# jhqxxx/aha

Hardware: AMD Instinct MI355X
Metric: decode tokens/s (greedy, batch 1) -- Qwen3-VL-8B, 1x1024^2 image + 512-token prompt; prefill tok/s alongside (higher is better)
Workload: dtype bf16; 1 GPU; qwen3vl8b; image=1024, kv_len_mid=2024, replicas=1, loop=device-resident greedy loop

## Files before the change

### aha_amd/_lib.py

```python
from __future__ import annotations

import ctypes as C
import os

_HERE = os.path.dirname(os.path.abspath(__file__))
LIB_PATH = os.path.join(_HERE, "csrc", "libaha_hip.so")

AHA_BF16, AHA_F16, AHA_F32, AHA_U32, AHA_U8 = 0, 1, 2, 3, 4
AHA_ARCH_QWEN3, AHA_ARCH_QWEN3VL, AHA_ARCH_QWEN3ASR = 0, 1, 2
ACT_NONE, ACT_GELU_TANH, ACT_GELU_ERF, ACT_SILU, ACT_SILU_MUL_PAIRS = 0, 1, 2, 3, 4


AHA_SAMPLE_HAS_TOP_P, AHA_SAMPLE_HAS_TOP_K = 1, 2
AHA_SAMPLE_NEED_LOGITS = 1


class SamplingParams(C.Structure):
    _fields_ = [
        ("temperature", C.c_float), ("top_p", C.c_float), ("top_k", C.c_int32), ("repeat_penalty", C.c_float),
        ("repeat_last_n", C.c_int32), ("flags", C.c_uint32), ("seed", C.c_uint64),
    ]


AHA_ENGINE_EV_FIRST, AHA_ENGINE_EV_STOP, AHA_ENGINE_EV_LENGTH, AHA_ENGINE_EV_CANCELLED = 1, 2, 4, 8
# ... 117 lines not shown
                                            C.c_int64]),
    "aha_hip_debug_resample_taps": (C.c_int64, [C.c_int32, C.c_int32, C.POINTER(C.c_float), C.c_int64, C.POINTER(C.c_int32),
                                                C.POINTER(C.c_int32)]),
    "aha_hip_audio_resample": (C.c_int64, [_P, C.POINTER(C.c_float), C.c_int64, C.c_int32, C.c_int32, C.c_int32,
                                           C.POINTER(C.c_float), C.c_int64]),
    "aha_hip_cache_len": (C.c_size_t, [_P]),
    "aha_hip_debug_steps_executed": (C.c_int64, [_P]),
    "aha_hip_debug_graph_step": (C.c_int, [_P, C.c_int32, C.POINTER(C.c_double), C.POINTER(C.c_double)]),
    "aha_hip_kv_export": (C.c_int, [_P, _P, C.c_size_t, C.POINTER(C.c_size_t), C.POINTER(C.c_size_t), C.POINTER(C.c_int64)]),
    "aha_hip_kv_import": (C.c_int, [_P, _P, C.c_size_t, C.c_int32, C.c_int32, C.c_int32, C.c_int32, C.c_size_t, C.c_int64]),
    "aha_hip_set_profiling": (C.c_int, [_P, C.c_int]),
    "aha_hip_get_profile": (C.c_int, [_P, C.c_char_p, C.POINTER(C.c_double), C.POINTER(C.c_int64),
                                      C.POINTER(C.c_double), C.POINTER(C.c_double)]),
    "aha_hip_debug_scramble_pages": (C.c_int, [_P, C.c_int]),
    "aha_hip_debug_attn_decode_form": (C.c_int, [_P]),
    "aha_hip_debug_last_hidden": (C.c_int, [_P, C.POINTER(C.c_float), C.c_size_t]),
    "aha_hip_debug_image_embeds": (C.c_int, [_P, C.c_int, C.POINTER(C.c_float), C.c_size_t]),
    "aha_hip_rmsnorm": (C.c_int, [_P, _P, _P, C.c_int64, C.c_int32, C.c_float, _P]),
    "aha_hip_gemv": (C.c_int, [_P, _P, _P, C.c_int32, C.c_int32, _P, C.c_float, _P, _P]),
    "aha_hip_gemv_gate_up": (C.c_int, [_P, _P, _P, _P, C.c_int32, C.c_int32, _P, C.c_float, _P]),
    "aha_hip_gemm": (C.c_int, [_P, _P, _P, C.c_int32, C.c_int32, C.c_int32, C.c_int32, C.c_int32, C.c_int32, _P, _P,
                               C.c_int32, _P]),
    "aha_hip_qknorm_rope": (C.c_int, [_P, _P, _P, _P, _P, _P, _P, _P, C.c_int32, C.c_int32, C.c_int32, C.c_int32,
                                      C.c_float, C.c_float, _P]),
    "aha_hip_attn_decode": (C.c_int, [_P, _P, _P, _P, C.c_int32, C.c_int32, C.c_int32, C.c_int32, C.c_float, _P]),
    "aha_hip_attn_prefill": (C.c_int, [_P, _P, _P, _P, C.c_int32, C.c_int32, C.c_int32, C.c_int32, C.c_int32,
                                       C.c_int32, C.c_int32, C.c_float, _P]),
    "aha_hip_debug_attn_prefill_segs": (C.c_int, [_P, _P, _P, _P, C.c_int32, C.c_int32, _P, C.c_int32, C.c_int32, C.c_float, _P]),
    "aha_hip_debug_prefill_rope": (C.c_int, [_P, _P, _P, _P, _P, _P, _P, C.c_int32, C.c_int32, C.c_int32, C.c_int32, C.c_int32, C.c_float,
                                             C.c_int32, C.c_int32, C.c_int32, _P, _P, C.c_int32, _P, _P, _P]),
# ... 121 lines not shown
```

### aha_amd/csrc/attn_decode_body.h

```cpp
#pragma once
#include <type_traits>
#include "attn_common.h"

namespace aha {

constexpr int ATTN_DECODE_NW = 4;
constexpr int ATTN_DECODE_MO_ROW = 132;
constexpr int ATTN_DECODE_FUSED_LDS = 16 * 128 * 2 + 128 * 2 + 128 * 2 + ATTN_DECODE_NW * 16 * ATTN_DECODE_MO_ROW * 4 + 2 * ATTN_DECODE_NW * 16 * 4;

__device__ __forceinline__ float split_sum16(const float (&v)[16]) {
#pragma clang fp contract(off)
  float t[8];
#pragma unroll
  for (int j = 0; j < 8; ++j) t[j] = v[j] + v[j + 8];
#pragma unroll
  for (int j = 0; j < 4; ++j) t[j] = t[j] + t[j + 4];
  const float c0 = t[0] + t[2], c1 = t[1] + t[3];
  return c0 + c1;
}

template <bool APPEND = true, bool LINEAR = false>
__device__ __forceinline__ bool attn_decode_fused_body(const AttnDecodeFusedArgs& a, char* smem, const int kvhd, const int split,
                                                       const int nsplit) {
  constexpr int NW = ATTN_DECODE_NW, NT = NW * 64;
  bf16_t* qs = reinterpret_cast<bf16_t*>(smem);
  bf16_t* ksn = qs + 16 * 128;
  bf16_t* vsn = ksn + 128;
  constexpr int MO_ROW = ATTN_DECODE_MO_ROW, MO_WAVE = 16 * MO_ROW;
  float* mo = reinterpret_cast<float*>(vsn + 128);
  float* mm = mo + NW * MO_WAVE;
  float* mlz = mm + NW * 16;
  const int tid = (int)threadIdx.x;
  const int wave = __builtin_amdgcn_readfirstlane(tid >> 6);
  const int lane = tid & 63, G = lane >> 4, c = lane & 15;
  const int g = a.nh / a.kvh;
  const int nunits = nsplit * NW, unit = split * NW + wave;
  const int L = a.kv_len_v, slot_new = a.kv_start_v;
  const int L_old = L - 1;
  const int npages = (L_old + KV_PAGE_TOKENS - 1) / KV_PAGE_TOKENS;

  const int tslot = (kvhd == 0 && split == 0) ? 0 : (kvhd == 0 && split == nsplit - 1 ? 1 : -1);
  auto stamp = [&](int k) {
    if (a.trace != nullptr && tslot >= 0 && tid == 0) a.trace[tslot * 6 + k] = wall_clock64();
  };
  stamp(0);

  const bf16_t* qkv = (const bf16_t*)a.qkv;
  const bool p_is_k = wave == g;
  const bool p_have = wave <= g;
  const bf16_t* p_src = p_is_k ? qkv + (int64_t)(a.nh + kvhd) * 128 : qkv + (int64_t)(kvhd * g + min(wave, g - 1)) * 128;
  const bf16_t* p_nw = (const bf16_t*)(p_is_k ? a.k_norm_w : a.q_norm_w);
  const bf16_t px0 = p_src[lane], px1 = p_src[lane + 64];
  const bf16_t pw0 = p_nw[lane], pw1 = p_nw[lane + 64];
  const float cs = a.rope[lane], sn = a.rope[64 + lane];
  bf16_t vnew = 0;
  if (tid < 128) vnew = qkv[(int64_t)(a.nh + a.kvh + kvhd) * 128 + tid];

  u32x4_t kf[4][4], vf[8][2];
  typedef const __attribute__((address_space(1))) char* gchar_t;
  const uint32_t l_off = (uint32_t)lane * 16;
  auto load_k = [&](uint64_t base) {
    gchar_t kb = reinterpret_cast<gchar_t>(base + (uint64_t)kvhd * KV_PAGE_TOKENS * 256);
#pragma unroll
    for (int sub = 0; sub < 4; ++sub)
#pragma unroll
      for (int k4 = 0; k4 < 4; ++k4)
        kf[sub][k4] = __builtin_nontemporal_load(reinterpret_cast<gptr16_t>(kb + (sub * 4 + k4) * 1024 + l_off));
  };
  auto load_v = [&](uint64_t base) {
    gchar_t vb = reinterpret_cast<gchar_t>(base + (uint64_t)a.kvh * KV_PAGE_TOKENS * 256 + (uint64_t)kvhd * 128 * (KV_PAGE_TOKENS * 2));
#pragma unroll
    for (int ds = 0; ds < 8; ++ds)
#pragma unroll
      for (int kk = 0; kk < 2; ++kk)
        vf[ds][kk] = __builtin_nontemporal_load(reinterpret_cast<gptr16_t>(vb + (ds * 2 + kk) * 1024 + l_off));
  };
  uint64_t my_pages = 0;
  auto fetch_page_ptrs = [&](int first_it) {
    if (LINEAR) return;
    const int pg = unit + (first_it + lane) * nunits;
    my_pages = pg < npages ? (uint64_t)(a.kv.page_ptrs[pg] + a.kv.layer_off) : 0;
  };
  auto page_base = [&](int i) {
    if (LINEAR) return a.lin_page0 + (uint64_t)((int64_t)(unit + i * nunits) * a.lin_step);
    const uint32_t lo = __builtin_amdgcn_readlane((uint32_t)my_pages, i & 63), hi = __builtin_amdgcn_readlane((uint32_t)(my_pages >> 32), i & 63);
    return ((uint64_t)hi << 32) | lo;
  };
  fetch_page_ptrs(0);
  int page = unit, it = 0;
  if (page < npages) {
    const uint64_t b0 = page_base(0);
    __builtin_amdgcn_sched_barrier(0);
    load_k(b0);
    __builtin_amdgcn_sched_barrier(0);
    load_v(b0);
    __builtin_amdgcn_sched_barrier(0);
  }

  {
    auto norm_rope = [&](bf16_t bx0, bf16_t bx1, bf16_t bw0, bf16_t bw1, bf16_t* dst) {
      float x0 = bf2f(bx0), x1 = bf2f(bx1);
      const float ss = wave_sum(fmaf(x0, x0, x1 * x1));
      const float rinv = 1.0f / sqrtf(ss / 128.0f + a.eps);
      x0 = rbf(x0 * rinv * bf2f(bw0));
      x1 = rbf(x1 * rinv * bf2f(bw1));
      const bf16_t y0 = f2bf(rbf(x0 * cs) + rbf(-x1 * sn));
      const bf16_t y1 = f2bf(rbf(x1 * cs) + rbf(x0 * sn));
      dst[lane] = y0;
      dst[lane + 64] = y1;
    };
    if (p_have) norm_rope(px0, px1, pw0, pw1, p_is_k ? ksn : qs + wave * 128);
    for (int hs = wave + NW; hs <= g; hs += NW) {
      const bool is_k = hs == g;
      const bf16_t* src = is_k ? qkv + (int64_t)(a.nh + kvhd) * 128 : qkv + (int64_t)(kvhd * g + hs) * 128;
      const bf16_t* nw = (const bf16_t*)(is_k ? a.k_norm_w : a.q_norm_w);
      norm_rope(src[lane], src[lane + 64], nw[lane], nw[lane + 64], is_k ? ksn : qs + hs * 128);
    }
    if (tid < 128) vsn[tid] = vnew;
  }
  __syncthreads();
  stamp(1);
  if (APPEND && split == 0) {
    typedef __attribute__((address_space(1))) bf16_t* gbf_t;
    const int pg = slot_new / KV_PAGE_TOKENS, t = slot_new % KV_PAGE_TOKENS;
    const uint64_t base = LINEAR ? a.lin_page0 + (uint64_t)((int64_t)pg * a.lin_step) : (uint64_t)(a.kv.page_ptrs[pg] + a.kv.layer_off);
    gbf_t kd = reinterpret_cast<gbf_t>(base) + (int64_t)kvhd * KV_PAGE_TOKENS * 128;
    gbf_t vd = reinterpret_cast<gbf_t>(base) + (int64_t)a.kvh * KV_PAGE_TOKENS * 128 + (int64_t)kvhd * 128 * KV_PAGE_TOKENS;
    for (int i = tid; i < 128; i += NT) {
      kd[kpage_elem(t, i, 4)] = ksn[i];
      vd[vpage_elem(t, i)] = vsn[i];
    }
  }

  bf16x8_t qf[4];
#pragma unroll
  for (int k4 = 0; k4 < 4; ++k4) {
    u32x4_t v = *reinterpret_cast<const u32x4_t*>(qs + min(c, g - 1) * 128 + k4 * 32 + G * 8);
    if (c >= g) v = u32x4_t{0u, 0u, 0u, 0u};
    qf[k4] = as_frag(v);
  }
  float m = -INFINITY, l = 0.f;
  f32x4_t o[8];
#pragma unroll
// ... 20 lines not shown
    float alpha;
    bf16x8_t pf[2];
    const int t0 = page * KV_PAGE_TOKENS;
    softmax_tile(st, a.scale, [&](int t) { return t0 + t < L_old; }, G, m, l, alpha, pf);
#pragma unroll
    for (int ds = 0; ds < 8; ++ds) {
      o[ds] *= alpha;
#pragma unroll
      for (int kk = 0; kk < 2; ++kk) o[ds] = mfma16(as_frag(vf[ds][kk]), pf[kk], o[ds]);
    }
    __builtin_amdgcn_sched_barrier(0);
    if (MORE) load_v(nb);
    __builtin_amdgcn_sched_barrier(0);
    page += nunits;
  };
  if (page < npages) {
    while (page + nunits < npages) do_page(std::true_type{});
    do_page(std::false_type{});
  }
  stamp(2);
  if (unit == 0) {
    float dot = 0.f;
    const u32x4_t* qr = reinterpret_cast<const u32x4_t*>(qs + min(c, g - 1) * 128 + G * 32);
    const u32x4_t* kr = reinterpret_cast<const u32x4_t*>(ksn + G * 32);
    u32x4_t qv[4], kv4[4];
#pragma unroll
    for (int j = 0; j < 4; ++j) {
      qv[j] = qr[j];
      kv4[j] = kr[j];
    }
#pragma unroll
    for (int j = 0; j < 16; ++j) {
      const uint32_t qw = qv[j >> 2][j & 3], kw = kv4[j >> 2][j & 3];
      dot = fmaf(__uint_as_float(qw << 16), __uint_as_float(kw << 16), dot);
      dot = fmaf(__uint_as_float(qw & 0xffff0000u), __uint_as_float(kw & 0xffff0000u), dot);
    }
// ... 2 lines not shown
    const float m_new = fmaxf(m, s);
    const float alpha = __expf(m - m_new);
    const float p = rbf(__expf(s - m_new));
    l = l * alpha + (G == 0 ? __expf(s - m_new) : 0.f);
    m = m_new;
#pragma unroll
    for (int ds = 0; ds < 8; ++ds) {
      const uint2 vv = *reinterpret_cast<const uint2*>(vsn + ds * 16 + G * 4);
      o[ds][0] = fmaf(p, __uint_as_float(vv.x << 16), o[ds][0] * alpha);
      o[ds][1] = fmaf(p, __uint_as_float(vv.x & 0xffff0000u), o[ds][1] * alpha);
      o[ds][2] = fmaf(p, __uint_as_float(vv.y << 16), o[ds][2] * alpha);
      o[ds][3] = fmaf(p, __uint_as_float(vv.y & 0xffff0000u), o[ds][3] * alpha);
    }
  }
  l = group_sum(l);

  {
    float* wo = mo + wave * MO_WAVE + c * MO_ROW + G * 4;
#pragma unroll
    for (int ds = 0; ds < 8; ++ds) *reinterpret_cast<f32x4_t*>(wo + ds * 16) = o[ds];
    if (G == 0) {
      mm[wave * 16 + c] = m;
      mlz[wave * 16 + c] = l;
    }
  }
  __syncthreads();
  const bool single = nsplit == 1;
  const auto rsrc_w = __builtin_amdgcn_make_buffer_rsrc(a.part_o, 0, (int)((size_t)nsplit * a.nh * 128 * 4), 0x00020000);
  for (int item = tid; item < g * 32; item += NT) {
    const int q = item >> 5, d0 = (item & 31) * 4;
// ... 155 lines not shown
```

### aha_amd/csrc/capi.hip

```cpp
#include <math.h>
#include <string.h>

#include <algorithm>
#include <map>
#include <memory>
#include <mutex>
#include <numeric>
#include <vector>

#include "common.h"
#include "model.h"
#include "sampler.h"
#include "audio.h"
#include "vision.h"

namespace aha {
const char* last_error_cstr();
}
using namespace aha;

#define API_GUARD_BEGIN try {
#define API_GUARD_END                                   \
  }                                                     \
  catch (const std::exception& e) {                     \
// ... 147 lines not shown
}

int aha_hip_last_logits(aha_model* m, float* logits_out) {
  API_GUARD_BEGIN
  if (!m || !logits_out) {
    set_error("null argument");
    return AHA_ERR_INVALID;
  }
  return model_last_logits(m, logits_out);
  API_GUARD_END
}

size_t aha_hip_cache_len(const aha_model* m) { return m ? m->cache_len : 0; }
int64_t aha_hip_debug_steps_executed(const aha_model* m) { return m ? m->steps_executed : 0; }
int aha_hip_debug_attn_decode_form(const aha_model* m) { return m ? m->last_attn_form : -1; }
int aha_hip_debug_graph_step(aha_model* m, int32_t replays, double* us_launches, double* us_graph) {
  if (!m) return AHA_ERR_INVALID;
  API_GUARD_BEGIN
  if (int rc = engine_owns_cache(m, "debug_graph_step")) return rc;
  return model_debug_graph_step(m, replays, us_launches, us_graph);
  API_GUARD_END
}
int aha_hip_kv_export(aha_model* m, void* out_dev, size_t out_bytes, size_t* bytes_needed, size_t* n_tokens, int64_t* rope_delta) {
  if (!m) return AHA_ERR_INVALID;
  API_GUARD_BEGIN
  if (int rc = engine_owns_cache(m, "kv_export")) return rc;
  return model_kv_export(m, out_dev, out_bytes, bytes_needed, n_tokens, rope_delta);
  API_GUARD_END
}
int aha_hip_kv_import(aha_model* m, const void* in_dev, size_t in_bytes, int32_t src_heads, int32_t src_head0, int32_t dst_head0, int32_t n_heads,
// ... 1593 lines not shown
```

### aha_amd/csrc/kernels.h

```cpp
#pragma once
#include <hip/hip_runtime.h>
#include <stdint.h>

#include <algorithm>
#include <utility>
#include <vector>

namespace aha {

struct KvLayer {
  const uint64_t* page_ptrs;
  uint64_t layer_off;
  int kvh, d;
};

enum GemvEpi { GEMV_STORE = 0, GEMV_RESIDUAL = 1, GEMV_SILU_MUL = 2, GEMV_LOGITS = 3, GEMV_PARTIAL_F32 = 4 };

struct GemvArgs {
  const void* W;
  const void* W2;
  const void* x;
  const void* norm_w;
  const void* residual;
  void* y;
// ... 89 lines not shown
  const void* k_norm_w;
  const float* rope;
  KvLayer kv;
  uint64_t lin_page0 = 0;
  int64_t lin_step = 0;
  int kv_start_v;
  int kv_len_v;
  float* part_o;
  float* part_ml;
  void* o;
  unsigned* head_ctr;
  unsigned ctr_target;
  unsigned long long* trace;
  int nh, kvh, nsplit;
  float eps, scale;
};
void launch_attn_decode_fused(const AttnDecodeFusedArgs& a, hipStream_t st);

struct AttnPrefillArgs {
  const void* q;
  KvLayer kv;
  void* o;
  int S, nh, kvh, d;
  int kv_offset;
  int kv_total;
  int causal;
  float scale;
  int64_t q_ld;
  int nqb;
  int S2 = 0, kv_offset2 = 0, kv_total2 = 0;
  int epi_rows = 0;
// ... 200 lines not shown
```

### aha_amd/csrc/kernels_attn.hip

```cpp
#include <stdio.h>
#include <stdlib.h>

#include "attn_decode_body.h"

namespace aha {

namespace {

template <int DQK, int DV, int QT, int NWV, bool TRACE = false, int ABL = 0, int SMX = 0>
__global__ __launch_bounds__(NWV * 64) __attribute__((amdgpu_waves_per_eu((NWV == 8 || DQK < 128) ? 4 : 3, 4))) void attn_prefill_kernel(AttnPrefillArgs a, unsigned long long* trace = nullptr) {
  constexpr int KS = DQK / 32, DS = DV / 16;
  constexpr bool LSUM = SMX == 3 && DQK == 96 && DV == 80;
  constexpr int RING = (DQK >= 128) ? 6 : 4;
  extern __shared__ __attribute__((aligned(16))) char smem[];
  const int tid = threadIdx.x, lane = tid & 63, wave = tid >> 6, G = lane >> 4, c = lane & 15;
  int head, qblk, seg_rows = a.S, seg_off = a.kv_offset, seg_tot = a.kv_total, seg_row0 = 0, page0 = 0;
  if (a.seg_tab != nullptr) {
    int it;
    if (a.nqb > 0) {
      const int xcd = blockIdx.x & 7, slot = blockIdx.x >> 3;
      const int g = a.nh / a.kvh, hpx = a.nh >> 3;
      const int hq = slot % hpx;
      head = (xcd + 8 * (hq / g)) * g + hq % g;
      it = slot / hpx;
// ... 432 lines not shown
    for (int j = 0; j < 8; ++j) acc += sw[u + j] * v[j];
  }
  for (; u < nunits; ++u) acc += sw[u] * po[u * ustride];
  ((bf16_t*)a.o)[head * 128 + d] = f2bf(acc / lsum);
}

struct AttnDecodeFusedTail {
  float* part_o;
  float* part_ml;
  void* o;
  unsigned* head_ctr;
  unsigned long long* trace;
  unsigned ctr_target;
  int kv_start_v, kv_kvh, kv_d;
  float eps, scale;
};

template <bool TRACE, bool LINEAR>
__device__ __forceinline__ void attn_decode_fused_flat(const void* qkv, uint64_t pages, uint64_t pages2, const float* rope,
                                                       const void* q_norm_w, const void* k_norm_w, int kv_len_v, int dims,
                                                       const AttnDecodeFusedTail& t, char* smem) {
  AttnDecodeFusedArgs a;
  a.qkv = qkv; a.q_norm_w = q_norm_w; a.k_norm_w = k_norm_w; a.rope = rope;
  a.kv.page_ptrs = LINEAR ? nullptr : reinterpret_cast<const uint64_t*>(pages); a.kv.layer_off = LINEAR ? 0 : pages2;
  a.lin_page0 = LINEAR ? pages : 0; a.lin_step = LINEAR ? (int64_t)pages2 : 0;
  a.kv.kvh = t.kv_kvh; a.kv.d = t.kv_d;
  a.kv_start_v = t.kv_start_v; a.kv_len_v = kv_len_v;
  a.part_o = t.part_o; a.part_ml = t.part_ml; a.o = t.o; a.head_ctr = t.head_ctr; a.ctr_target = t.ctr_target;
  a.trace = TRACE ? t.trace : nullptr;
  a.nh = dims & 1023; a.kvh = (dims >> 10) & 1023; a.nsplit = dims >> 20; a.eps = t.eps; a.scale = t.scale;
  attn_decode_fused_body<true, LINEAR>(a, smem, (int)blockIdx.x, (int)blockIdx.y, a.nsplit);
}

#define AHA_ATTN_DECODE_FUSED_KERNEL(NAME, TRACE, LINEAR)                                                                                    \
  __global__ __launch_bounds__(256, 2) void NAME(const void* qkv, uint64_t pages, uint64_t pages2, const float* rope, const void* q_norm_w, \
                                                 const void* k_norm_w, int kv_len_v, int dims, AttnDecodeFusedTail t) {                      \
    __shared__ __attribute__((aligned(16))) char smem[ATTN_DECODE_FUSED_LDS];                                                                \
    attn_decode_fused_flat<TRACE, LINEAR>(qkv, pages, pages2, rope, q_norm_w, k_norm_w, kv_len_v, dims, t, smem);                            \
  }
AHA_ATTN_DECODE_FUSED_KERNEL(attn_decode_fused_kernel, false, true)
AHA_ATTN_DECODE_FUSED_KERNEL(attn_decode_fused_table_kernel, false, false)
AHA_ATTN_DECODE_FUSED_KERNEL(attn_decode_fused_traced_kernel, true, true)
AHA_ATTN_DECODE_FUSED_KERNEL(attn_decode_fused_table_traced_kernel, true, false)
#undef AHA_ATTN_DECODE_FUSED_KERNEL

}

void launch_attn_decode_fused(const AttnDecodeFusedArgs& a, hipStream_t st) {
  const AttnDecodeFusedTail t{a.part_o, a.part_ml, a.o, a.head_ctr, a.trace, a.ctr_target, a.kv_start_v, a.kv.kvh, a.kv.d, a.eps, a.scale};
  if (a.nh > 1023 || a.kvh > 1023 || a.nsplit > 1024 || a.nsplit < 1) {
    fprintf(stderr, "launch_attn_decode_fused: head / split counts out of range\n");
    abort();
  }
  const int dims = a.nh | (a.kvh << 10) | (a.nsplit << 20);
  const bool linear = a.lin_step != 0;
  const uint64_t pages = linear ? a.lin_page0 : (uint64_t)(uintptr_t)a.kv.page_ptrs;
  const uint64_t pages2 = linear ? (uint64_t)a.lin_step : a.kv.layer_off;
  auto kernel = a.trace == nullptr ? (linear ? attn_decode_fused_kernel : attn_decode_fused_table_kernel)
                                   : (linear ? attn_decode_fused_traced_kernel : attn_decode_fused_table_traced_kernel);
  hipLaunchKernelGGL(kernel, dim3(a.kvh, a.nsplit), dim3(256), 0, st, a.qkv, pages, pages2, a.rope, a.q_norm_w, a.k_norm_w, a.kv_len_v,
                     dims, t);
}

static int g_attn_smx_override = -1;
void set_attn_variant_override(int smx) { g_attn_smx_override = smx; }
static int g_attn_form_override = -1;
void set_attn_form_override(int form) { g_attn_form_override = form; }

static int attn_prefill_form(const AttnPrefillArgs& a, int smx);
static int attn_prefill_smx(const AttnPrefillArgs& a);
static int attn_prefill_smx(const AttnPrefillArgs& a) {
  static const int smx_env = [] { const char* e = getenv("AHA_ATTN_SMX"); return e ? atoi(e) : 3; }();
// ... 126 lines not shown
```

### aha_amd/csrc/model.h

```cpp
#pragma once
#include <hip/hip_runtime.h>

#include <map>
#include <string>
#include <vector>

#include "../../include/aha_hip.h"
#include "kernels.h"

struct aha_ctx {
  int device = 0;
  hipStream_t stream = nullptr;
};

namespace aha {

void set_error(const std::string& msg);
#define AHA_HIP_CHECK(expr)                                                                          \
  do {                                                                                               \
    hipError_t _e = (expr);                                                                          \
    if (_e != hipSuccess) {                                                                          \
      ::aha::set_error(std::string(#expr) + " failed: " + hipGetErrorString(_e));                    \
      return AHA_ERR_HIP;                                                                            \
    }                                                                                                \
// ... 49 lines not shown
  int32_t* d_axis_map = nullptr;
  float* d_rope = nullptr;
  float attn_scale = 0.f;
  std::vector<void*> slabs;
  std::vector<uint64_t> h_page_ptrs;
  uint64_t* d_page_ptrs = nullptr;
  size_t page_table_cap = 0;
  size_t pages_per_slab = 0;
  uint64_t page_bytes = 0;
  uint64_t layer_stride = 0;
  size_t n_pages = 0;
  size_t lin_pages = 0;
  uint64_t lin_p0 = 0;
  int64_t lin_step = 0;
  int last_attn_form = -1;
  size_t cache_len = 0;
  bool scramble_pages = false;
  std::vector<uint64_t> free_pages;
  aha::StepState* d_state = nullptr;
  aha::StepState* h_state = nullptr;
  uint32_t* d_token_log = nullptr;
  size_t token_log_cap = 0;
  uint32_t* h_ring = nullptr;
  uint32_t* h_ring_dev = nullptr;
  uint32_t* h_done = nullptr;
  uint32_t* h_done_dev = nullptr;
  int64_t steps_executed = 0;
  bool rope_delta_valid = false;
  int64_t rope_delta = 0;
  void *d_x = nullptr, *d_qkv = nullptr, *d_q = nullptr, *d_attn = nullptr, *d_act = nullptr, *d_hlast = nullptr;
// ... 155 lines not shown
```

### aha_amd/csrc/model.hip

```cpp
#include "model.h"

#include <math.h>
#include <stdlib.h>
#include <string.h>

#include <algorithm>
#include <chrono>
#include <deque>

#include "common.h"
#include "audio.h"
#include "sampler.h"
#include "vision.h"

namespace aha {

static thread_local std::string g_last_error;
void set_error(const std::string& msg) { g_last_error = msg; }
const char* last_error_cstr() { return g_last_error.c_str(); }

ProfScope::ProfScope(aha_model* m_, const char* cls, double bytes, double flops) : m(m_) {
  if (!m->profiling) return;
  auto it = m->prof_cls.find(cls);
  int c;
// ... 819 lines not shown
}

static int fetch_outputs(aha_model* m, float* logits_out, uint32_t* argmax_out) {
  const aha_model_desc& c = m->desc;
  m->have_logits = true;
  m->logits_assembled = false;
  if (logits_out) {
    const int rc = assemble_logits(m);
    if (rc) return rc;
  }
  if (logits_out) AHA_HIP_CHECK(hipMemcpyAsync(m->h_logits, m->d_logits, (size_t)c.vocab_size * 4, hipMemcpyDeviceToHost, m->stream));
  AHA_HIP_CHECK(hipMemcpyAsync(&m->h_state->next_token, &m->d_state->next_token, 4, hipMemcpyDeviceToHost, m->stream));
  AHA_HIP_CHECK(hipStreamSynchronize(m->stream));
  if (m->d_gemv_trace) gemv_trace_dump(m);
  if (m->d_attn_trace) {
    const int L = m->desc.num_hidden_layers;
    std::vector<unsigned long long> t((size_t)L * 12);
    if (hipMemcpy(t.data(), m->d_attn_trace, t.size() * 8, hipMemcpyDeviceToHost) == hipSuccess) {
      for (int b = 0; b < 2; ++b) {
        double v[5] = {};
        int n = 0;
        for (int li = 1; li < L; ++li) {
          const unsigned long long* p = t.data() + (size_t)li * 12 + b * 6;
          if (p[0] == 0 || p[4] == 0) continue;
          for (int k = 0; k < 5; ++k) v[k] += (p[k + 1] > p[k] ? (double)(p[k + 1] - p[k]) : 0.0) * 0.01;
          ++n;
        }
        if (n) fprintf(stderr, "[attn trace] block %d: prologue %.2f | pages %.2f | merge+publish %.2f | arrive %.2f | final merge %.2f us\n", b, v[0] / n, v[1] / n, v[2] / n, v[3] / n, v[4] / n);
      }
      double dstart = 0.0, arr[2] = {};
      int n = 0;
      for (int li = 1; li < L; ++li) {
        const unsigned long long* p = t.data() + (size_t)li * 12;
        if (p[0] == 0 || p[4] == 0 || p[6] == 0 || p[10] == 0) continue;
        const unsigned long long t0 = std::min(p[0], p[6]);
        dstart += ((double)p[6] - (double)p[0]) * 0.01;
        arr[0] += (double)(p[4] - t0) * 0.01;
        arr[1] += (double)(p[10] - t0) * 0.01;
        ++n;
      }
      if (n) fprintf(stderr, "[attn trace] start of block 1 - start of block 0 %+.2f | arrival after the earlier start: block 0 %.2f | block 1 %.2f us\n", dstart / n, arr[0] / n, arr[1] / n);
    }
  }
  if (logits_out) memcpy(logits_out, m->h_logits, (size_t)c.vocab_size * 4);
  if (argmax_out) *argmax_out = m->h_state->next_token;
  return AHA_OK;
}


int model_allreduce(aha_model* m, float* buf, size_t count) {
  if (m->tp_size <= 1) return AHA_OK;
  ProfScope ps(m, "allreduce", (double)count * 4, 0);
  if (m->rccl_comm) return rccl_allreduce(m, buf, count);
  if (!m->allreduce_cb) {
    set_error("tp_size > 1 but no all-reduce was installed (aha_hip_set_allreduce / aha_hip_tp_init_rccl)");
    return AHA_ERR_STATE;
// ... 407 lines not shown
static void enqueue_decode_step(aha_model* m, size_t kv_len_after, bool embed = true, bool tail = false) {
  const aha_model_desc& c = m->desc;
  const int H = c.hidden_size, I = c.intermediate_size, d = c.head_dim, nh = c.num_attention_heads, kvh = c.num_key_value_heads;
  const int nq = nh * d, nkv = kvh * d;
  hipStream_t st = m->stream;
  if (embed) {
    ProfScope ps(m, "elem", H * 4.0, 0);
    hipLaunchKernelGGL(embed_state_kernel, dim3(1), dim3(256), 0, st, (const bf16_t*)m->embed, m->d_state, (bf16_t*)m->d_x, H,
                       m->d_inv_freq, m->d_axis_map, m->d_rope);
  }
  const int npages = (int)((kv_len_after + KV_PAGE_TOKENS - 1) / KV_PAGE_TOKENS);
  static const char* e_div = getenv("AHA_ATTN_PAGES_PER_BLOCK");
  const int div = e_div ? std::max(1, atoi(e_div)) : 4;
  int nsplit = (npages + div - 1) / div;
  nsplit = std::max(1, std::min(std::min(nsplit, m->max_nsplit), 1024 / (nh / kvh)));
  for (int li = 0; li < c.num_hidden_layers; ++li) {
    const LayerWeights& L = m->layers[li];
    {
      GemvArgs g{};
      g.W = L.wqkv; g.x = m->d_x; g.norm_w = L.in_norm; g.eps = c.rms_norm_eps; g.y = m->d_qkv; g.N = nq + 2 * nkv; g.K = H;
      g.trace = gemv_trace_slot(m, li * 4 + 0);
      ProfScope ps(m, "gemv", (double)g.N * g.K * 2 + g.K * 4.0 + g.N * 2.0, 2.0 * g.N * g.K);
      launch_gemv(g, GEMV_STORE, st);
    }
    if (m->decode_fused) {
      AttnDecodeFusedArgs a{};
      a.qkv = m->d_qkv; a.q_norm_w = L.q_norm; a.k_norm_w = L.k_norm; a.rope = m->d_rope;
      a.kv = model_kv_layer(m, li); a.kv_start_v = (int)kv_len_after - 1; a.kv_len_v = (int)kv_len_after;
      if ((size_t)npages <= m->lin_pages && !m->scramble_pages) {
        a.lin_page0 = m->lin_p0 + a.kv.layer_off;
        a.lin_step = m->lin_step;
      }
      m->last_attn_form = a.lin_step != 0 ? 1 : 0;
      a.part_o = m->d_part_o; a.part_ml = m->d_part_ml; a.nh = nh; a.kvh = kvh; a.nsplit = nsplit; a.eps = c.rms_norm_eps;
      a.scale = m->attn_scale; a.o = m->d_attn; a.head_ctr = m->d_bar + DECODE_HEAD_CTR_WORD;
      if (nsplit > 1) m->head_ctr_base += (unsigned)nsplit;
      a.ctr_target = m->head_ctr_base;
      static const char* e_at = getenv("AHA_ATTN_TRACE");
      if (e_at && atoi(e_at)) {
        if (!m->d_attn_trace) {
          void* tp = nullptr;
          if (dev_alloc(m, (size_t)c.num_hidden_layers * 12 * 8, &tp, true) == AHA_OK) m->d_attn_trace = (unsigned long long*)tp;
        }
        if (m->d_attn_trace) a.trace = m->d_attn_trace + (size_t)li * 12;
      }
      GemvArgs g{};
      g.W = L.wo; g.x = m->d_attn; g.residual = m->d_x; g.y = m->d_x; g.N = H; g.K = nq;
      g.trace = gemv_trace_slot(m, li * 4 + 1);
      const double attn_bytes = (double)kv_len_after * 2 * nkv * 2 + (nq + 2 * nkv) * 2.0 + nsplit * nq * 4.0;
      const double gemv_bytes = (double)g.N * g.K * 2 + g.K * 2.0 + g.N * 4.0;
      {
        ProfScope ps(m, "attn_decode", attn_bytes, 4.0 * kv_len_after * nq);
        launch_attn_decode_fused(a, st);
      }
      ProfScope ps(m, "gemv", gemv_bytes, 2.0 * g.N * g.K);
      gemv_row_parallel(m, g);
    } else {
      {
        RopeArgs r{};
// ... 2126 lines not shown
```

### aha_amd/model.py

```python
from __future__ import annotations

import ctypes as C
import os
import time
from dataclasses import dataclass
from typing import Dict, List, Optional, Sequence

import numpy as np
import torch

from . import _lib
from ._lib import MmInput, ModelDesc, TensorView, check, lib
from .configs import Qwen3ASRConfig, Qwen3Config, Qwen3VLConfig

_DT = {torch.bfloat16: _lib.AHA_BF16, torch.float16: _lib.AHA_F16, torch.float32: _lib.AHA_F32}


class HipContext:
    def __init__(self, device: int = 0):
        self.handle = C.c_void_p()
        check(lib().aha_hip_init(device, C.byref(self.handle)))
        self.device = device

    def close(self):
# ... 494 lines not shown

    def debug_steps_executed(self) -> int:
        return int(lib().aha_hip_debug_steps_executed(self.handle))

    def set_profiling(self, on: bool):
        check(lib().aha_hip_set_profiling(self.handle, int(on)))

    def get_profile(self, kernel_class: str):
        ms, n, b, f = C.c_double(), C.c_int64(), C.c_double(), C.c_double()
        check(lib().aha_hip_get_profile(self.handle, kernel_class.encode(), C.byref(ms), C.byref(n), C.byref(b), C.byref(f)))
        return {"ms": ms.value, "launches": n.value, "bytes": b.value, "flops": f.value}

    def debug_attn_decode_form(self) -> int:
        return int(lib().aha_hip_debug_attn_decode_form(self.handle))

    def debug_scramble_pages(self, on: bool = True):
        check(lib().aha_hip_debug_scramble_pages(self.handle, int(on)))

    def debug_last_hidden(self) -> np.ndarray:
        out = np.empty(self.text_cfg.hidden_size, dtype=np.float32)
        check(lib().aha_hip_debug_last_hidden(self.handle, out.ctypes.data_as(C.POINTER(C.c_float)), out.size))
        return out

    def debug_image_embeds(self, which: int, rows: int) -> np.ndarray:
        out = np.empty((rows, self.text_cfg.hidden_size), dtype=np.float32)
        check(lib().aha_hip_debug_image_embeds(self.handle, which, out.ctypes.data_as(C.POINTER(C.c_float)), out.size))
        return out

    def vision_encode(self, data: "MultiModalData") -> torch.Tensor:
        mm = MmInput()
# ... 276 lines not shown
```

### include/aha_hip.h

```cpp
#ifndef AHA_HIP_H
#define AHA_HIP_H

#include <stddef.h>
#include <stdint.h>

#ifdef __cplusplus
extern "C" {
#endif

typedef struct aha_ctx aha_ctx;
typedef struct aha_model aha_model;

enum aha_status {
  AHA_OK = 0,
  AHA_ERR_INVALID = -1,
  AHA_ERR_HIP = -2,
  AHA_ERR_OOM = -3,
  AHA_ERR_SHAPE = -4,
  AHA_ERR_MISSING_WEIGHT = -5,
  AHA_ERR_UNSUPPORTED = -6,
  AHA_ERR_STATE = -7
};

enum aha_dtype { AHA_BF16 = 0, AHA_F16 = 1, AHA_F32 = 2, AHA_U32 = 3, AHA_U8 = 4 };
// ... 248 lines not shown
int aha_hip_cp_init_rccl(aha_model* m, const void* unique_id128);
int aha_hip_debug_cp_plan(int32_t n_tokens, int32_t world, int32_t rank, int32_t* out5);
int aha_hip_kv_export(aha_model* m, void* out_dev, size_t out_bytes, size_t* bytes_needed, size_t* n_tokens, int64_t* rope_delta);
int aha_hip_kv_import(aha_model* m, const void* in_dev, size_t in_bytes, int32_t src_heads, int32_t src_head0, int32_t dst_head0,
                      int32_t n_heads, size_t n_tokens, int64_t rope_delta);
int aha_hip_debug_allreduce(aha_model* m, void* buf_f32_dev, size_t count);

size_t aha_hip_cache_len(const aha_model* m);
int64_t aha_hip_debug_steps_executed(const aha_model* m);
int aha_hip_debug_graph_step(aha_model* m, int32_t replays, double* us_launches, double* us_graph);
int aha_hip_set_profiling(aha_model* m, int enable);
int aha_hip_get_profile(aha_model* m, const char* kernel_class, double* total_ms, int64_t* launches, double* bytes,
                        double* flops);
int aha_hip_debug_scramble_pages(aha_model* m, int enable);
int aha_hip_debug_attn_decode_form(const aha_model* m);
int aha_hip_debug_last_hidden(aha_model* m, float* out, size_t n);
int aha_hip_debug_poison_lds(uint32_t seed, void* stream);
int aha_hip_debug_gemm_grouped(const void* A, const void* W, void* C, int32_t M, int32_t N, int32_t K, int32_t ldc, int32_t act,
                               int32_t groups, int32_t a_gstride, int32_t c_gstride, int32_t c_row0, int32_t m_total, void* stream);
int aha_hip_debug_attn_variant(int32_t smx);
int aha_hip_debug_attn_form(int32_t form);
int aha_hip_debug_gemm_plan(int32_t tile, int32_t splitk);
int aha_hip_debug_plan_gemm(int32_t M, int32_t N, int32_t K, int32_t act, int32_t has_bias, int32_t has_residual, size_t workspace_bytes,
                            int32_t* out3);
int aha_hip_debug_streamk_plan(int32_t M, int32_t N, int32_t K, int32_t tile_n, int32_t workers, size_t workspace_bytes, int32_t* out,
                               int32_t cap, int32_t* off_out, int32_t* info7);
int aha_hip_set_gemm_reserved_cus(int32_t n);
int aha_hip_debug_image_embeds(aha_model* m, int which , float* out, size_t n);

int aha_hip_rmsnorm(const void* x, const void* w, void* y, int64_t rows, int32_t dim, float eps, void* stream);
// ... 73 lines not shown
```

Baseline: 341.7 tokens/s.

## Add per-wave unit form of fused decode attention spreading pages across more blocks

Adds a UNIT variant of the fused decode attention kernel. Each block handles one page-unit: only wave 0 walks pages, and the grid grows to kvh x units instead of kvh x nsplit. Each unit writes its own partial output and max/sum to global memory, and the last-arriving block merges them through a templated multi-split merge. This aims to spread the KV page work over more CUs and use less LDS per block, at the cost of more blocks, more partials to merge and more atomics. It is on by default when nsplit is between 2 and 8, and AHA_ATTN_SPREAD=0 turns it off.

```diff
diff --git a/aha_amd/_lib.py b/aha_amd/_lib.py
--- a/aha_amd/_lib.py
+++ b/aha_amd/_lib.py
@@ -155,6 +155,7 @@
                                       C.POINTER(C.c_double), C.POINTER(C.c_double)]),
     "aha_hip_debug_scramble_pages": (C.c_int, [_P, C.c_int]),
     "aha_hip_debug_attn_decode_form": (C.c_int, [_P]),
+    "aha_hip_debug_attn_decode_units": (C.c_int, [_P]),
     "aha_hip_debug_last_hidden": (C.c_int, [_P, C.POINTER(C.c_float), C.c_size_t]),
     "aha_hip_debug_image_embeds": (C.c_int, [_P, C.c_int, C.POINTER(C.c_float), C.c_size_t]),
     "aha_hip_rmsnorm": (C.c_int, [_P, _P, _P, C.c_int64, C.c_int32, C.c_float, _P]),
diff --git a/aha_amd/csrc/attn_decode_body.h b/aha_amd/csrc/attn_decode_body.h
--- a/aha_amd/csrc/attn_decode_body.h
+++ b/aha_amd/csrc/attn_decode_body.h
@@ -19,9 +19,147 @@
   return c0 + c1;
 }
 
-template <bool APPEND = true, bool LINEAR = false>
+constexpr int ATTN_DECODE_UNIT_MAX_SPLITS = 8;
+constexpr int ATTN_DECODE_UNIT_LDS = 16 * 128 * 2 + 128 * 2 + 128 * 2 + 16;
+
+template <int NS>
+__device__ __forceinline__ void attn_decode_unit_merge(const AttnDecodeFusedArgs& a, float2* pairs_lds, const int kvhd, const int g,
+                                                       const int nlaunch, const int tid) {
+  constexpr int NU = NS * 4, NT = ATTN_DECODE_NW * 64;
+  const auto rsrc = __builtin_amdgcn_make_buffer_rsrc(a.part_o, 0, (int)((size_t)NU * a.nh * 128 * 4), 0x00020000);
+  uint32_t unit_stride = (uint32_t)a.nh * 128 * 4;
+  int last_unit = nlaunch - 1;
+  asm volatile("" : "+v"(unit_stride), "+v"(last_unit));
+  for (int item = tid; item < g * 32; item += NT) {
+    const int head = kvhd * g + (item >> 5);
+    float2* prow = pairs_lds + (tid >> 5) * 32;
+    const float2 pmine = act_ldf2<true>(a.part_ml + ((size_t)min(item & 31, last_unit) * a.nh + head) * 2);
+    const uint32_t off = (uint32_t)(head * 128 + (item & 31) * 4) * 4;
+    f32x4_t pv[NU];
+#pragma unroll
+    for (int u = 0; u < NU; ++u) {
+      const u32x4_t v = __builtin_amdgcn_raw_buffer_load_b128(rsrc, off + (uint32_t)(u < NU - 4 ? u : min(u, last_unit)) * unit_stride, 0, 16 );
+      pv[u] = f32x4_t{__uint_as_float(v[0]), __uint_as_float(v[1]), __uint_as_float(v[2]), __uint_as_float(v[3])};
+    }
+    prow[item & 31] = pmine;
+    __builtin_amdgcn_wave_barrier();
+    float2 ml[NU];
+#pragma unroll
+    for (int u = 0; u < NU; ++u) ml[u] = prow[u];
+    __builtin_amdgcn_wave_barrier();
+    float sm[NS], sl[NS];
+    f32x4_t so[NS];
+#pragma unroll
+    for (int s = 0; s < NS; ++s) {
+      float mu[4], lu[4];
+      f32x4_t ou[4];
+#pragma unroll
+      for (int w = 0; w < 4; ++w) {
+        const int u = s * 4 + w;
+        const bool active = s < NS - 1 || u < nlaunch;
+        mu[w] = active ? ml[u].x : -INFINITY;
+        lu[w] = active ? ml[u].y : 0.f;
+#pragma unroll
+        for (int e = 0; e < 4; ++e) ou[w][e] = active ? pv[u][e] : 0.f;
+      }
+      float M = -INFINITY;
+#pragma unroll
+      for (int w = 0; w < 4; ++w) M = fmaxf(M, mu[w]);
+      float acc[4] = {0.f, 0.f, 0.f, 0.f}, ls = 0.f;
+#pragma unroll
+      for (int w = 0; w < 4; ++w) {
+        const float wt = (mu[w] == -INFINITY) ? 0.f : __expf(mu[w] - M);
+#pragma unroll
+        for (int e = 0; e < 4; ++e) acc[e] = fmaf(wt, ou[w][e], acc[e]);
+        ls = fmaf(wt, lu[w], ls);
+      }
+      sm[s] = M;
+      sl[s] = ls;
+      so[s] = f32x4_t{acc[0], acc[1], acc[2], acc[3]};
+    }
+    float M = -INFINITY;
+#pragma unroll
+    for (int j = 0; j < NS; ++j) M = fmaxf(M, sm[j]);
+    float wgt[16], wl[16];
+#pragma unroll
+    for (int j = 0; j < 16; ++j) {
+      float lj = sl[j < NS ? j : NS - 1];
+      if (j < NS) {
+        wgt[j] = (sm[j] != -INFINITY) ? __expf(sm[j] - M) : 0.f;
+      } else {
+        asm volatile("v_mov_b32 %0, 0" : "=v"(wgt[j]));
+        asm volatile("" : "+v"(lj));
+      }
+      wl[j] = fmaf(wgt[j], lj, 0.f);
+    }
+    const float inv = 1.0f / split_sum16(wl);
+    f32x4_t f = {0.f, 0.f, 0.f, 0.f};
+#pragma unroll
+    for (int j = 0; j < 16; ++j)
+#pragma unroll
+      for (int e = 0; e < 4; ++e) f[e] = fmaf(wgt[j], so[j < NS ? j : NS - 1][e], f[e]);
+    uint2 w;
+    w.x = pack_bf(f[0] * inv, f[1] * inv);
+    w.y = pack_bf(f[2] * inv, f[3] * inv);
+    *reinterpret_cast<uint2*>((bf16_t*)a.o + (kvhd * g) * 128 + item * 4) = w;
+  }
+}
+
+template <typename Stamp>
+__device__ __forceinline__ bool attn_decode_unit_tail(const AttnDecodeFusedArgs& a, float2* pairs_lds, int* s_last, const int kvhd, const int unit,
+                                                      const int nlaunch, const int nsplit, const float m, const float l,
+                                                      const f32x4_t (&o)[8], Stamp stamp) {
+  const int tid = (int)threadIdx.x;
+  const int wave = __builtin_amdgcn_readfirstlane(tid >> 6);
+  const int lane = tid & 63, G = lane >> 4, c = lane & 15;
+  const int g = a.nh / a.kvh;
+  if (wave == 0) {
+    if (c < g) {
+      const auto rsrc_w = __builtin_amdgcn_make_buffer_rsrc(a.part_o, 0, (int)((size_t)nsplit * 4 * a.nh * 128 * 4), 0x00020000);
+      const int head = kvhd * g + c;
+      const uint32_t off = (uint32_t)(((size_t)unit * a.nh + head) * 128 + G * 4) * 4;
+#pragma unroll
+      for (int ds = 0; ds < 8; ++ds) {
+        const u32x4_t v = {__float_as_uint(o[ds][0]), __float_as_uint(o[ds][1]), __float_as_uint(o[ds][2]), __float_as_uint(o[ds][3])};
+        __builtin_amdgcn_raw_buffer_store_b128(v, rsrc_w, off + ds * 64, 0, 16 );
+      }
+      if (G == 0) {
+        const unsigned long long mlp = ((unsigned long long)__float_as_uint(l) << 32) | __float_as_uint(m);
+        __hip_atomic_store(reinterpret_cast<unsigned long long*>(a.part_ml + ((int64_t)unit * a.nh + head) * 2), mlp, __ATOMIC_RELAXED,
+                           __HIP_MEMORY_SCOPE_AGENT);
+      }
+    }
+    stamp(3);
+    asm volatile("s_waitcnt vmcnt(0)" ::: "memory");
+    if (lane == 0) {
+      const unsigned prev = __hip_atomic_fetch_add(a.head_ctr + 32 * kvhd, 1u, __ATOMIC_RELAXED, __HIP_MEMORY_SCOPE_AGENT);
+      *s_last = (prev + 1u == a.ctr_target) ? 1 : 0;
+    }
+  }
+  __syncthreads();
+  stamp(4);
+  if (*s_last == 0) return false;
+#define AHA_UNIT_MERGE_CASE(NS)                                        \
+  if (nsplit == NS) {                                                  \
+    attn_decode_unit_merge<NS>(a, pairs_lds, kvhd, g, nlaunch, tid);   \
+    stamp(5);                                                          \
+    return true;                                                       \
+  }
+  AHA_UNIT_MERGE_CASE(7)
+  AHA_UNIT_MERGE_CASE(8)
+  AHA_UNIT_MERGE_CASE(6)
+  AHA_UNIT_MERGE_CASE(5)
+  AHA_UNIT_MERGE_CASE(4)
+  AHA_UNIT_MERGE_CASE(3)
+#undef AHA_UNIT_MERGE_CASE
+  attn_decode_unit_merge<2>(a, pairs_lds, kvhd, g, nlaunch, tid);
+  stamp(5);
+  return true;
+}
+
+template <bool APPEND = true, bool LINEAR = false, bool UNIT = false>
 __device__ __forceinline__ bool attn_decode_fused_body(const AttnDecodeFusedArgs& a, char* smem, const int kvhd, const int split,
-                                                       const int nsplit) {
+                                                       const int nsplit, const int nlaunch = 0) {
   constexpr int NW = ATTN_DECODE_NW, NT = NW * 64;
   bf16_t* qs = reinterpret_cast<bf16_t*>(smem);
   bf16_t* ksn = qs + 16 * 128;
@@ -34,12 +172,15 @@
   const int wave = __builtin_amdgcn_readfirstlane(tid >> 6);
   const int lane = tid & 63, G = lane >> 4, c = lane & 15;
   const int g = a.nh / a.kvh;
-  const int nunits = nsplit * NW, unit = split * NW + wave;
+  const int nunits = nsplit * NW, unit = UNIT ? split : split * NW + wave;
+  const bool pager = !UNIT || wave == 0;
+  const bool need_kv = !UNIT || unit == 0;
   const int L = a.kv_len_v, slot_new = a.kv_start_v;
   const int L_old = L - 1;
   const int npages = (L_old + KV_PAGE_TOKENS - 1) / KV_PAGE_TOKENS;
 
-  const int tslot = (kvhd == 0 && split == 0) ? 0 : (kvhd == 0 && split == nsplit - 1 ? 1 : -1);
+  const int tlast = UNIT ? nlaunch - 1 : nsplit - 1;
+  const int tslot = kvhd != 0 ? -1 : split == 0 ? 0 : split == tlast ? 1 : split == 1 ? 2 : -1;
   auto stamp = [&](int k) {
     if (a.trace != nullptr && tslot >= 0 && tid == 0) a.trace[tslot * 6 + k] = wall_clock64();
   };
@@ -47,14 +188,14 @@
 
   const bf16_t* qkv = (const bf16_t*)a.qkv;
   const bool p_is_k = wave == g;
-  const bool p_have = wave <= g;
+  const bool p_have = wave < g || (p_is_k && need_kv);
   const bf16_t* p_src = p_is_k ? qkv + (int64_t)(a.nh + kvhd) * 128 : qkv + (int64_t)(kvhd * g + min(wave, g - 1)) * 128;
   const bf16_t* p_nw = (const bf16_t*)(p_is_k ? a.k_norm_w : a.q_norm_w);
   const bf16_t px0 = p_src[lane], px1 = p_src[lane + 64];
   const bf16_t pw0 = p_nw[lane], pw1 = p_nw[lane + 64];
   const float cs = a.rope[lane], sn = a.rope[64 + lane];
   bf16_t vnew = 0;
-  if (tid < 128) vnew = qkv[(int64_t)(a.nh + a.kvh + kvhd) * 128 + tid];
+  if (tid < 128 && need_kv) vnew = qkv[(int64_t)(a.nh + a.kvh + kvhd) * 128 + tid];
 
   u32x4_t kf[4][4], vf[8][2];
   typedef const __attribute__((address_space(1))) char* gchar_t;
@@ -77,7 +218,7 @@
   };
   uint64_t my_pages = 0;
   auto fetch_page_ptrs = [&](int first_it) {
-    if (LINEAR) return;
+    if (LINEAR || !pager) return;
     const int pg = unit + (first_it + lane) * nunits;
     my_pages = pg < npages ? (uint64_t)(a.kv.page_ptrs[pg] + a.kv.layer_off) : 0;
   };
@@ -88,7 +229,7 @@
   };
   fetch_page_ptrs(0);
   int page = unit, it = 0;
-  if (page < npages) {
+  if (pager && page < npages) {
     const uint64_t b0 = page_base(0);
     __builtin_amdgcn_sched_barrier(0);
     load_k(b0);
@@ -112,11 +253,12 @@
     if (p_have) norm_rope(px0, px1, pw0, pw1, p_is_k ? ksn : qs + wave * 128);
     for (int hs = wave + NW; hs <= g; hs += NW) {
       const bool is_k = hs == g;
+      if (UNIT && is_k && !need_kv) break;
       const bf16_t* src = is_k ? qkv + (int64_t)(a.nh + kvhd) * 128 : qkv + (int64_t)(kvhd * g + hs) * 128;
       const bf16_t* nw = (const bf16_t*)(is_k ? a.k_norm_w : a.q_norm_w);
       norm_rope(src[lane], src[lane + 64], nw[lane], nw[lane + 64], is_k ? ksn : qs + hs * 128);
     }
-    if (tid < 128) vsn[tid] = vnew;
+    if (tid < 128 && need_kv) vsn[tid] = vnew;
   }
   __syncthreads();
   stamp(1);
@@ -126,7 +268,8 @@
     const uint64_t base = LINEAR ? a.lin_page0 + (uint64_t)((int64_t)pg * a.lin_step) : (uint64_t)(a.kv.page_ptrs[pg] + a.kv.layer_off);
     gbf_t kd = reinterpret_cast<gbf_t>(base) + (int64_t)kvhd * KV_PAGE_TOKENS * 128;
     gbf_t vd = reinterpret_cast<gbf_t>(base) + (int64_t)a.kvh * KV_PAGE_TOKENS * 128 + (int64_t)kvhd * 128 * KV_PAGE_TOKENS;
-    for (int i = tid; i < 128; i += NT) {
+    for (int i = UNIT ? tid - 64 : tid; i < 128; i += NT) {
+      if (UNIT && i < 0) continue;
       kd[kpage_elem(t, i, 4)] = ksn[i];
       vd[vpage_elem(t, i)] = vsn[i];
     }
@@ -177,12 +320,12 @@
     __builtin_amdgcn_sched_barrier(0);
     page += nunits;
   };
-  if (page < npages) {
+  if (pager && page < npages) {
     while (page + nunits < npages) do_page(std::true_type{});
     do_page(std::false_type{});
   }
   stamp(2);
-  if (unit == 0) {
+  if (unit == 0 && pager) {
     float dot = 0.f;
     const u32x4_t* qr = reinterpret_cast<const u32x4_t*>(qs + min(c, g - 1) * 128 + G * 32);
     const u32x4_t* kr = reinterpret_cast<const u32x4_t*>(ksn + G * 32);
@@ -215,6 +358,7 @@
     }
   }
   l = group_sum(l);
+  if constexpr (UNIT) return attn_decode_unit_tail(a, reinterpret_cast<float2*>(qs), reinterpret_cast<int*>(vsn + 128), kvhd, unit, nlaunch, nsplit, m, l, o, stamp);
 
   {
     float* wo = mo + wave * MO_WAVE + c * MO_ROW + G * 4;
diff --git a/aha_amd/csrc/capi.hip b/aha_amd/csrc/capi.hip
--- a/aha_amd/csrc/capi.hip
+++ b/aha_amd/csrc/capi.hip
@@ -185,6 +185,7 @@
 size_t aha_hip_cache_len(const aha_model* m) { return m ? m->cache_len : 0; }
 int64_t aha_hip_debug_steps_executed(const aha_model* m) { return m ? m->steps_executed : 0; }
 int aha_hip_debug_attn_decode_form(const aha_model* m) { return m ? m->last_attn_form : -1; }
+int aha_hip_debug_attn_decode_units(const aha_model* m) { return m ? m->last_attn_units : -1; }
 int aha_hip_debug_graph_step(aha_model* m, int32_t replays, double* us_launches, double* us_graph) {
   if (!m) return AHA_ERR_INVALID;
   API_GUARD_BEGIN
diff --git a/aha_amd/csrc/kernels.h b/aha_amd/csrc/kernels.h
--- a/aha_amd/csrc/kernels.h
+++ b/aha_amd/csrc/kernels.h
@@ -127,7 +127,9 @@
   unsigned long long* trace;
   int nh, kvh, nsplit;
   float eps, scale;
-};
+  int units = 0;
+};
+constexpr int ATTN_TRACE_WORDS = 18;
 void launch_attn_decode_fused(const AttnDecodeFusedArgs& a, hipStream_t st);
 
 struct AttnPrefillArgs {
diff --git a/aha_amd/csrc/kernels_attn.hip b/aha_amd/csrc/kernels_attn.hip
--- a/aha_amd/csrc/kernels_attn.hip
+++ b/aha_amd/csrc/kernels_attn.hip
@@ -470,9 +470,10 @@
   unsigned ctr_target;
   int kv_start_v, kv_kvh, kv_d;
   float eps, scale;
+  int units;
 };
 
-template <bool TRACE, bool LINEAR>
+template <bool TRACE, bool LINEAR, bool UNIT = false>
 __device__ __forceinline__ void attn_decode_fused_flat(const void* qkv, uint64_t pages, uint64_t pages2, const float* rope,
                                                        const void* q_norm_w, const void* k_norm_w, int kv_len_v, int dims,
                                                        const AttnDecodeFusedTail& t, char* smem) {
@@ -485,25 +486,30 @@
   a.part_o = t.part_o; a.part_ml = t.part_ml; a.o = t.o; a.head_ctr = t.head_ctr; a.ctr_target = t.ctr_target;
   a.trace = TRACE ? t.trace : nullptr;
   a.nh = dims & 1023; a.kvh = (dims >> 10) & 1023; a.nsplit = dims >> 20; a.eps = t.eps; a.scale = t.scale;
-  attn_decode_fused_body<true, LINEAR>(a, smem, (int)blockIdx.x, (int)blockIdx.y, a.nsplit);
-}
-
-#define AHA_ATTN_DECODE_FUSED_KERNEL(NAME, TRACE, LINEAR)                                                                                    \
+  attn_decode_fused_body<true, LINEAR, UNIT>(a, smem, (int)blockIdx.x, (int)blockIdx.y, a.nsplit, UNIT ? t.units : 0);
+}
+
+#define AHA_ATTN_DECODE_FUSED_KERNEL(NAME, TRACE, LINEAR, UNIT)                                                                              \
   __global__ __launch_bounds__(256, 2) void NAME(const void* qkv, uint64_t pages, uint64_t pages2, const float* rope, const void* q_norm_w, \
                                                  const void* k_norm_w, int kv_len_v, int dims, AttnDecodeFusedTail t) {                      \
-    __shared__ __attribute__((aligned(16))) char smem[ATTN_DECODE_FUSED_LDS];                                                                \
-    attn_decode_fused_flat<TRACE, LINEAR>(qkv, pages, pages2, rope, q_norm_w, k_norm_w, kv_len_v, dims, t, smem);                            \
-  }
-AHA_ATTN_DECODE_FUSED_KERNEL(attn_decode_fused_kernel, false, true)
-AHA_ATTN_DECODE_FUSED_KERNEL(attn_decode_fused_table_kernel, false, false)
-AHA_ATTN_DECODE_FUSED_KERNEL(attn_decode_fused_traced_kernel, true, true)
-AHA_ATTN_DECODE_FUSED_KERNEL(attn_decode_fused_table_traced_kernel, true, false)
+    __shared__ __attribute__((aligned(16))) char smem[UNIT ? ATTN_DECODE_UNIT_LDS : ATTN_DECODE_FUSED_LDS];                                  \
+    attn_decode_fused_flat<TRACE, LINEAR, UNIT>(qkv, pages, pages2, rope, q_norm_w, k_norm_w, kv_len_v, dims, t, smem);                      \
+  }
+AHA_ATTN_DECODE_FUSED_KERNEL(attn_decode_fused_kernel, false, true, false)
+AHA_ATTN_DECODE_FUSED_KERNEL(attn_decode_fused_table_kernel, false, false, false)
+AHA_ATTN_DECODE_FUSED_KERNEL(attn_decode_fused_traced_kernel, true, true, false)
+AHA_ATTN_DECODE_FUSED_KERNEL(attn_decode_fused_table_traced_kernel, true, false, false)
+AHA_ATTN_DECODE_FUSED_KERNEL(attn_decode_unit_kernel, false, true, true)
+AHA_ATTN_DECODE_FUSED_KERNEL(attn_decode_unit_table_kernel, false, false, true)
+AHA_ATTN_DECODE_FUSED_KERNEL(attn_decode_unit_traced_kernel, true, true, true)
+AHA_ATTN_DECODE_FUSED_KERNEL(attn_decode_unit_table_traced_kernel, true, false, true)
 #undef AHA_ATTN_DECODE_FUSED_KERNEL
 
 }
 
 void launch_attn_decode_fused(const AttnDecodeFusedArgs& a, hipStream_t st) {
-  const AttnDecodeFusedTail t{a.part_o, a.part_ml, a.o, a.head_ctr, a.trace, a.ctr_target, a.kv_start_v, a.kv.kvh, a.kv.d, a.eps, a.scale};
+  const AttnDecodeFusedTail t{a.part_o, a.part_ml, a.o, a.head_ctr, a.trace, a.ctr_target, a.kv_start_v, a.kv.kvh, a.kv.d, a.eps, a.scale,
+                              a.units};
   if (a.nh > 1023 || a.kvh > 1023 || a.nsplit > 1024 || a.nsplit < 1) {
     fprintf(stderr, "launch_attn_decode_fused: head / split counts out of range\n");
     abort();
@@ -512,6 +518,18 @@
   const bool linear = a.lin_step != 0;
   const uint64_t pages = linear ? a.lin_page0 : (uint64_t)(uintptr_t)a.kv.page_ptrs;
   const uint64_t pages2 = linear ? (uint64_t)a.lin_step : a.kv.layer_off;
+  if (a.units != 0) {
+    if (a.nsplit < 2 || a.nsplit > ATTN_DECODE_UNIT_MAX_SPLITS || a.units < 1 || a.units > a.nsplit * ATTN_DECODE_NW ||
+        a.units <= (a.nsplit - 1) * ATTN_DECODE_NW - 1) {
+      fprintf(stderr, "launch_attn_decode_fused: unit form outside its split / unit counts\n");
+      abort();
+    }
+    auto kernel = a.trace == nullptr ? (linear ? attn_decode_unit_kernel : attn_decode_unit_table_kernel)
+                                     : (linear ? attn_decode_unit_traced_kernel : attn_decode_unit_table_traced_kernel);
+    hipLaunchKernelGGL(kernel, dim3(a.kvh, a.units), dim3(256), 0, st, a.qkv, pages, pages2, a.rope, a.q_norm_w, a.k_norm_w, a.kv_len_v,
+                       dims, t);
+    return;
+  }
   auto kernel = a.trace == nullptr ? (linear ? attn_decode_fused_kernel : attn_decode_fused_table_kernel)
                                    : (linear ? attn_decode_fused_traced_kernel : attn_decode_fused_table_traced_kernel);
   hipLaunchKernelGGL(kernel, dim3(a.kvh, a.nsplit), dim3(256), 0, st, a.qkv, pages, pages2, a.rope, a.q_norm_w, a.k_norm_w, a.kv_len_v,
diff --git a/aha_amd/csrc/model.h b/aha_amd/csrc/model.h
--- a/aha_amd/csrc/model.h
+++ b/aha_amd/csrc/model.h
@@ -87,6 +87,7 @@
   uint64_t lin_p0 = 0;
   int64_t lin_step = 0;
   int last_attn_form = -1;
+  int last_attn_units = -1;
   size_t cache_len = 0;
   bool scramble_pages = false;
   std::vector<uint64_t> free_pages;
diff --git a/aha_amd/csrc/model.hip b/aha_amd/csrc/model.hip
--- a/aha_amd/csrc/model.hip
+++ b/aha_amd/csrc/model.hip
@@ -857,32 +857,39 @@
   AHA_HIP_CHECK(hipStreamSynchronize(m->stream));
   if (m->d_gemv_trace) gemv_trace_dump(m);
   if (m->d_attn_trace) {
-    const int L = m->desc.num_hidden_layers;
-    std::vector<unsigned long long> t((size_t)L * 12);
+    const int L = m->desc.num_hidden_layers, W = ATTN_TRACE_WORDS;
+    std::vector<unsigned long long> t((size_t)L * W);
     if (hipMemcpy(t.data(), m->d_attn_trace, t.size() * 8, hipMemcpyDeviceToHost) == hipSuccess) {
-      for (int b = 0; b < 2; ++b) {
+      for (int b = 0; b < 3; ++b) {
         double v[5] = {};
         int n = 0;
         for (int li = 1; li < L; ++li) {
-          const unsigned long long* p = t.data() + (size_t)li * 12 + b * 6;
+          const unsigned long long* p = t.data() + (size_t)li * W + b * 6;
           if (p[0] == 0 || p[4] == 0) continue;
           for (int k = 0; k < 5; ++k) v[k] += (p[k + 1] > p[k] ? (double)(p[k + 1] - p[k]) : 0.0) * 0.01;
           ++n;
         }
         if (n) fprintf(stderr, "[attn trace] block %d: prologue %.2f | pages %.2f | merge+publish %.2f | arrive %.2f | final merge %.2f us\n", b, v[0] / n, v[1] / n, v[2] / n, v[3] / n, v[4] / n);
       }
-      double dstart = 0.0, arr[2] = {};
-      int n = 0;
+      double dstart[2] = {}, arr[3] = {};
+      int n = 0, n2 = 0;
       for (int li = 1; li < L; ++li) {
-        const unsigned long long* p = t.data() + (size_t)li * 12;
+        const unsigned long long* p = t.data() + (size_t)li * W;
         if (p[0] == 0 || p[4] == 0 || p[6] == 0 || p[10] == 0) continue;
-        const unsigned long long t0 = std::min(p[0], p[6]);
-        dstart += ((double)p[6] - (double)p[0]) * 0.01;
+        const bool mid = p[12] != 0 && p[16] != 0;
+        const unsigned long long t0 = std::min(std::min(p[0], p[6]), mid ? p[12] : p[0]);
+        dstart[0] += ((double)p[6] - (double)p[0]) * 0.01;
         arr[0] += (double)(p[4] - t0) * 0.01;
         arr[1] += (double)(p[10] - t0) * 0.01;
         ++n;
-      }
-      if (n) fprintf(stderr, "[attn trace] start of block 1 - start of block 0 %+.2f | arrival after the earlier start: block 0 %.2f | block 1 %.2f us\n", dstart / n, arr[0] / n, arr[1] / n);
+        if (mid) {
+          dstart[1] += ((double)p[12] - (double)p[0]) * 0.01;
+          arr[2] += (double)(p[16] - t0) * 0.01;
+          ++n2;
+        }
+      }
+      if (n) fprintf(stderr, "[attn trace] start of block 1 - start of block 0 %+.2f | arrival after the earliest start: block 0 %.2f | block 1 %.2f us\n", dstart[0] / n, arr[0] / n, arr[1] / n);
+      if (n2) fprintf(stderr, "[attn trace] start of block 2 - start of block 0 %+.2f | arrival after the earliest start: block 2 %.2f us\n", dstart[1] / n2, arr[2] / n2);
     }
   }
   if (logits_out) memcpy(logits_out, m->h_logits, (size_t)c.vocab_size * 4);
@@ -1320,6 +1327,10 @@
   const int div = e_div ? std::max(1, atoi(e_div)) : 4;
   int nsplit = (npages + div - 1) / div;
   nsplit = std::max(1, std::min(std::min(nsplit, m->max_nsplit), 1024 / (nh / kvh)));
+  static const char* e_spread = getenv("AHA_ATTN_SPREAD");
+  const int old_pages = (int)((kv_len_after - 1 + KV_PAGE_TOKENS - 1) / KV_PAGE_TOKENS);
+  int attn_units = std::min(nsplit * 4, std::max(1, old_pages));
+  if ((e_spread && atoi(e_spread) == 0) || nsplit < 2 || nsplit > 8 || attn_units < (nsplit - 1) * 4) attn_units = 0;
   for (int li = 0; li < c.num_hidden_layers; ++li) {
     const LayerWeights& L = m->layers[li];
     {
@@ -1338,17 +1349,19 @@
         a.lin_step = m->lin_step;
       }
       m->last_attn_form = a.lin_step != 0 ? 1 : 0;
+      m->last_attn_units = attn_units != 0 ? 1 : 0;
+      a.units = attn_units;
       a.part_o = m->d_part_o; a.part_ml = m->d_part_ml; a.nh = nh; a.kvh = kvh; a.nsplit = nsplit; a.eps = c.rms_norm_eps;
       a.scale = m->attn_scale; a.o = m->d_attn; a.head_ctr = m->d_bar + DECODE_HEAD_CTR_WORD;
-      if (nsplit > 1) m->head_ctr_base += (unsigned)nsplit;
+      if (nsplit > 1) m->head_ctr_base += (unsigned)(attn_units ? attn_units : nsplit);
       a.ctr_target = m->head_ctr_base;
       static const char* e_at = getenv("AHA_ATTN_TRACE");
       if (e_at && atoi(e_at)) {
         if (!m->d_attn_trace) {
           void* tp = nullptr;
-          if (dev_alloc(m, (size_t)c.num_hidden_layers * 12 * 8, &tp, true) == AHA_OK) m->d_attn_trace = (unsigned long long*)tp;
+          if (dev_alloc(m, (size_t)c.num_hidden_layers * ATTN_TRACE_WORDS * 8, &tp, true) == AHA_OK) m->d_attn_trace = (unsigned long long*)tp;
         }
-        if (m->d_attn_trace) a.trace = m->d_attn_trace + (size_t)li * 12;
+        if (m->d_attn_trace) a.trace = m->d_attn_trace + (size_t)li * ATTN_TRACE_WORDS;
       }
       GemvArgs g{};
       g.W = L.wo; g.x = m->d_attn; g.residual = m->d_x; g.y = m->d_x; g.N = H; g.K = nq;
diff --git a/aha_amd/model.py b/aha_amd/model.py
--- a/aha_amd/model.py
+++ b/aha_amd/model.py
@@ -532,6 +532,9 @@
     def debug_attn_decode_form(self) -> int:
         return int(lib().aha_hip_debug_attn_decode_form(self.handle))
 
+    def debug_attn_decode_units(self) -> int:
+        return int(lib().aha_hip_debug_attn_decode_units(self.handle))
+
     def debug_scramble_pages(self, on: bool = True):
         check(lib().aha_hip_debug_scramble_pages(self.handle, int(on)))
 
diff --git a/include/aha_hip.h b/include/aha_hip.h
--- a/include/aha_hip.h
+++ b/include/aha_hip.h
@@ -286,6 +286,7 @@
                         double* flops);
 int aha_hip_debug_scramble_pages(aha_model* m, int enable);
 int aha_hip_debug_attn_decode_form(const aha_model* m);
+int aha_hip_debug_attn_decode_units(const aha_model* m);
 int aha_hip_debug_last_hidden(aha_model* m, float* out, size_t n);
 int aha_hip_debug_poison_lds(uint32_t seed, void* stream);
 int aha_hip_debug_gemm_grouped(const void* A, const void* W, void* C, int32_t M, int32_t N, int32_t K, int32_t ldc, int32_t act,
```

After: 343.7 tokens/s, median of 6. Within noise of the previous version (+0.6%).
